# yl602019618/Reconstruction-of-PDE-without-Time-Label

Hardware: AMD Instinct MI355X
Metric: snapshot-bags/sec (train step) + rel-L2 drift error, 2D FPE 128² @1/2/4/8 GPU (higher is better)
Workload: dtype f32; 1 GPU; 2d_FPE train_fno.py NIOFP2D_FNO(2,3,100,25,3,12,32,2) (C), grid 128x128; per_gpu_batch=4, global_batch=4, T=100, bag_size=L=randint(50,T) with replacement, dataset_bags=4096, parallelism=dp1, optimizer=Adam lr 0.0005 (fused flat), launch=hip-graph per bag size L (all kernels replayed each step)

## Files before the change

include/blindno.h:

```cpp
#ifndef BLINDNO_H
#define BLINDNO_H

#include <stdint.h>

#ifdef __cplusplus
extern "C" {
#endif

typedef void* blindno_stream_t;

int blindno_abi_version(void);
const char* blindno_error_string(int code);


int blindno_lift_fwd(const float* in, const float* w0, const float* b0, float* x0,
                     int Bn, int N1, int N2, int Cin, int C, int P1, int P2,
                     blindno_stream_t stream);

int blindno_lift_bwd(const float* dx0, const float* in, const float* w0, float* d_in,
                     float* partial, int nchunk,
                     int Bn, int N1, int N2, int Cin, int C, int P1, int P2,
                     blindno_stream_t stream);
int blindno_lift_bwd_nchunk(int Bn, int N1, int N2);

int blindno_project_fwd(const float* z, const float* w1, const float* b1, const float* w2,
                        const float* b2, float* out, int Bn, int C, int P1, int P2, int Ho,
                        int Wo, int Hd, int Cout, int ostride, int ooff,
                        blindno_stream_t stream);

int blindno_project_bwd(const float* z, const float* w1, const float* b1, const float* w2,
                        const float* dout, float* dz, float* partial, int nchunk,
                        int Bn, int C, int P1, int P2, int Ho, int Wo, int Hd, int Cout,
                        int ostride, int ooff, int dout_div, blindno_stream_t stream);
int blindno_project_bwd_nchunk(int Bn, int Ho, int Wo);
int blindno_project_bwd_nchunk_heads(int Bg, int Ho, int Wo);
int blindno_project_bwd_w(const float* z, const float* w1, const float* b1, const float* w2,
                          const float* dout, const float* lscale, float* dz, float* partial,
                          int nchunk, int Bn, int C, int P1, int P2, int Ho, int Wo, int Hd,
                          int Cout, int ostride, int ooff, int dout_div, blindno_stream_t stream);

int64_t blindno_project_bag_stats_floats(int B, int Ho, int Wo);
int blindno_project_bag_bwd_nchunk(int B, int Ho, int Wo);
int blindno_project_bag_fwd(const float* z, const float* w1, const float* b1, const float* w2,
                            const float* b2, const float* lw, float* ubar, float* stats,
                            float* v, int B, int U, int C, int P1, int P2, int Ho, int Wo, int Hd,
                            blindno_stream_t stream);
int blindno_project_bag_bwd(const float* stats, const float* gs, const float* w2, const float* lw,
                            const float* v, float* dz, float* partial, int nchunk, int B, int U,
                            int C, int P1, int P2, int Ho, int Wo, int Hd,
                            blindno_stream_t stream);


int blindno_rowdft(const float* x, float* At, const float* Tp, int Bn, int C, int P1,
                   int P2, int m2, int act, blindno_stream_t stream);
int blindno_rowdft_crop(const float* x, float* At, const float* Tp, int Bn, int C, int P1,
                        int P2, int m2, int act, int N1v, int N2v, blindno_stream_t stream);

int blindno_colpass(const float* At, const float* Wt, float* Xs, float* Y, float* Z,
                    const float* FB, const float* GB, int Bn, int Ci, int Co, int P1, int m1,
                    int m2, int P2, int dir, blindno_stream_t stream);

int blindno_mix_wgrad_nsplit(int Bn, int Ci, int Co, int K1, int m2);
int blindno_mix_wgrad(const float* X, const float* G, float* dWt, float* partial, int nsplit,
                      int Bn, int Ci, int Co, int K1, int m2, blindno_stream_t stream);
int blindno_mix_wgrad_part(const float* X, const float* G, float* partial, int nsplit, int Gw,
                           int Bn, int Ci, int Co, int K1, int m2, blindno_stream_t stream);
int blindno_mix_wgrad_multi(const void* const* X, const void* const* G, void* const* out,
                            const int* shp, int njobs, blindno_stream_t stream);
int blindno_mix_wgrad_multi_u(const void* const* X, const void* const* G, void* const* out,
                              const int* shp, void* const* ud, const int* um1, int njobs,
                              blindno_stream_t stream);

int blindno_mix1d(const float* At, const float* Wt, float* Xs, float* Z, int Bn, int Ci,
                  int Co, int m, int P2, int dir, blindno_stream_t stream);

int blindno_rowidft_epi(const float* Z, const float* x, const float* wc, const float* bc,
                        float* z, const float* tb, int Bn, int C, int P1, int P2, int m2,
                        int act, blindno_stream_t stream);
int blindno_rowidft_epi_crop(const float* Z, const float* x, const float* wc, const float* bc,
                             float* z, const float* tb, int Bn, int C, int P1, int P2, int m2,
                             int act, int oN1, int oN2, blindno_stream_t stream);

int blindno_rowidft_bwd(const float* G, const float* dz, const float* wc, const float* xsrc,
                        float* dx, const float* tb, float* partial, int Bn, int C, int P1,
                        int P2, int m2, int act, blindno_stream_t stream);
int blindno_rowidft_bwd_crop(const float* G, const float* dz, const float* wc, const float* xsrc,
                             float* dx, const float* tb, float* partial, int Bn, int C, int P1,
                             int P2, int m2, int act, int dN1, int dN2, blindno_stream_t stream);
int blindno_rowidft_bwd_nchunk(int Bn, int C, int P1, int P2, int m2);
int blindno_set_rowfuse(int on);
int blindno_set_colfuse(int on);
int blindno_rowidft_bwd_rd(const float* G, const float* dz, const float* wc, const float* xsrc,
                           float* dx, const float* tb, float* partial, int Bn, int C, int P1,
                           int P2, int m2, int act, int dN1, int dN2, float* At, const float* Tp,
                           blindno_stream_t stream);
int blindno_rowidft_epi_rd(const float* Z, const float* x, const float* wc, const float* bc,
                           float* z, const float* tb, int Bn, int C, int P1, int P2, int m2,
                           int act, float* At, const float* Tp, int act_next,
                           blindno_stream_t stream);

int blindno_spectrum_tile_layout(int Bn, int C, int P1, int P2, int m2);


int blindno_rowdft_bag_lift(const float* X, const int* idx, const float* w0, const float* Gt,
                            float* At, const float* Tp, int B, int T, int L, int N1, int N2,
                            int C, int P1, int P2, int m2, blindno_stream_t stream);
int blindno_rowdft_bag_lift_dg(const float* X, const int* idx, const float* w0, const float* b0,
                               const float* Dg, float* At, const float* Tp, int B, int T, int L,
                               int N1, int N2, int C, int P1, int P2, int m2,
                               blindno_stream_t stream);

int blindno_rowidft_epi_lift(const float* Z, const float* X, const int* idx, const float* grid,
                             const float* w0, const float* b0, const float* wc, const float* bc,
                             float* z, const float* tb, int B, int T, int L, int N1, int N2,
                             int C, int P1, int P2, int m2, blindno_stream_t stream);
int blindno_rowidft_epi_lift_rd(const float* Z, const float* X, const int* idx, const float* grid,
                                const float* w0, const float* b0, const float* wc,
                                const float* bc, float* z, const float* tb, int B, int T, int L,
                                int N1, int N2, int C, int P1, int P2, int m2, float* At,
                                const float* Tp, int act_next, blindno_stream_t stream);

int blindno_rowidft_bwd_lift(const float* G, const float* dz, const float* X, const int* idx,
                             const float* grid, const float* w0, const float* b0, const float* wc,
                             const float* tb, float* partial, int B, int T, int L, int N1, int N2,
                             int C, int P1, int P2, int m2, blindno_stream_t stream);

int blindno_colspec_ok(int Bn, int C, int P1, int P2, int m1, int m2);
int blindno_colspec_nchunk(int C, int m2);
int blindno_colspec_bwd_nchunk(int Bn, int P1);
int blindno_rowdft_cd(const float* x, float* part, const float* Tp, const float* tab, int Bn, int C,
                      int P1, int P2, int m2, int act, int N1v, int N2v, blindno_stream_t stream);
int blindno_rowdft_bag_lift_cd(const float* X, const int* idx, float* part, const float* Tp,
                               const float* tab, int B, int T, int L, int N1, int N2, int P1,
                               int P2, int m2, blindno_stream_t stream);
int blindno_rowdft_bag_lift_cd_pack(const float* X, const int* idx, float* part, const float* Tp,
                                    const float* tab, int B, int T, int L, int N1, int N2, int P1,
                                    int P2, int m2, const void* const* w1s, const void* const* w2s,
                                    void* const* Wts, const int* shapes, int npk,
                                    blindno_stream_t stream);
int blindno_colmix(const float* part, int nbv, const float* Wt, float* Xsave, float* Y, int Bn, int C,
                   int Cp, int P1, int P2, int m1, int m2, int dir, const float* w0, const float* b0,
                   const float* Dg2, blindno_stream_t stream);
int blindno_rowidft_epi_zc(const float* Y, const float* x, const float* wc, const float* bc, float* z,
                           const float* tb, const float* tab, float* part, const float* Tp, int Bn,
                           int C, int P1, int P2, int m1, int m2, int act, int act_next, int oN1,
                           int oN2, blindno_stream_t stream);
int blindno_rowidft_epi_lift_zc(const float* Y, const float* X, const int* idx, const float* grid,
                                const float* w0, const float* b0, const float* wc, const float* bc,
                                float* z, const float* tb, const float* tab, float* part,
                                const float* Tp, int B, int T, int L, int N1, int N2, int C, int P1,
                                int P2, int m1, int m2, int act_next, blindno_stream_t stream);
int blindno_rowidft_bwd_zc(const float* Y, const float* dz, const float* wc, const float* xsrc,
                           float* dx, const float* tb, const float* tab, float* part,
                           const float* Tp, float* partial, int Bn, int C, int P1, int P2, int m1,
                           int m2, int act, int dN1, int dN2, blindno_stream_t stream);
int blindno_rowdft_cd_bag(const float* v, const float* ghat, const float* lw, int U, float* part,
                          const float* Tp, const float* tab, int Bn, int C, int P1, int P2, int m2,
                          int Ho, int Wo, blindno_stream_t stream);
int blindno_rowidft_bwd_zc_bag(const float* Y, const float* v, const float* ghat, const float* lw,
                               int U, const float* wc, const float* xsrc, float* dx, const float* tb,
                               const float* tab, float* part, const float* Tp, float* partial,
                               int Bn, int C, int P1, int P2, int m1, int m2, int act, int Ho, int Wo,
                               blindno_stream_t stream);
int blindno_rowidft_bwd_lift_zc_mix(const float* Y, const float* dz, const float* X, const int* idx,
                                    const float* grid, const float* w0, const float* b0,
                                    const float* wc, const float* tb, const float* tab,
                                    float* partial, int B, int T, int L, int N1, int N2, int C,
                                    int P1, int P2, int m1, int m2, const void* const* mX,
                                    const void* const* mG, void* const* mOut, const int* mshp,
                                    int nmj, blindno_stream_t stream);
int blindno_rowidft_bwd_lift_zc(const float* Y, const float* dz, const float* X, const int* idx,
                                const float* grid, const float* w0, const float* b0,
                                const float* wc, const float* tb, const float* tab, float* partial,
                                int B, int T, int L, int N1, int N2, int C, int P1, int P2, int m1,
                                int m2, blindno_stream_t stream);

int blindno_conv_wgrad(const float* dz, const float* x, float* partial, int nchunk, int Bn,
                       int C, int P1, int P2, int act, blindno_stream_t stream);
int blindno_conv_wgrad_nchunk(int Bn, int P1, int P2);

int blindno_reduce_partials(const float* partial, float* out, int nchunk, int np,
                            blindno_stream_t stream);

int blindno_reduce_partials_multi(const void* const* partials, void* const* outs,
                                  const int* nchunks, const int* nps, int nseg,
                                  blindno_stream_t stream);
int blindno_reduce_partials_pieces(const void* const* partials, void* const* outs,
                                   const int* nchunks, const int* nps, const int* e0s,
                                   const int* e1s, int nseg, blindno_stream_t stream);
int blindno_reduce_segs_limit(int what);
int blindno_reduce_partials_pieces_u(const void* const* partials, void* const* outs,
                                     const int* nchunks, const int* nps, const int* e0s,
                                     const int* e1s, const int* upks, void* const* ud,
                                     const int* ushp, int nseg, blindno_stream_t stream);
int blindno_finish_multi(const void* const* partials, void* const* outs, const int* nchunks,
                         const int* nps, const int* e0s, const int* e1s, const int* upks,
                         void* const* ud, const int* ushp, int nseg, const void* const* dWts,
                         void* const* dw1s, void* const* dw2s, const int* shapes, int nunp,
                         blindno_stream_t stream);
// ... 261 lines not shown
```

reconstruction-of-pde-without-time-label_amd/blindno/_lib.py:

```python
from __future__ import annotations

import ctypes
import os
import threading

import torch

_HERE = os.path.dirname(os.path.abspath(__file__))
LIB_PATH = os.environ.get("BLINDNO_LIB", os.path.join(_HERE, "libblindno.so"))

SIGNATURES = {
    "blindno_abi_version": "",
    "blindno_lift_fwd": "ppppiiiiiiis",
    "blindno_lift_bwd": "pppppiiiiiiiis",
    "blindno_project_fwd": "ppppppiiiiiiiiiis",
    "blindno_project_bwd": "pppppppiiiiiiiiiiiis",
    "blindno_rowdft": "pppiiiiiis",
    "blindno_rowdft_crop": "pppiiiiiiiis",
    "blindno_rowdft_bag_lift": "ppppppiiiiiiiiis",
    "blindno_rowdft_bag_lift_dg": "pppppppiiiiiiiiis",
    "blindno_rowidft_epi_lift": "ppppppppppiiiiiiiiis",
    "blindno_rowidft_bwd_lift": "ppppppppppiiiiiiiiis",
    "blindno_colpass": "pppppppiiiiiiiis",
    "blindno_colspec_ok": "iiiiii",
    "blindno_colspec_nchunk": "ii",
    "blindno_colspec_bwd_nchunk": "ii",
    "blindno_rowdft_cd": "ppppiiiiiiiis",
    "blindno_rowdft_bag_lift_cd": "pppppiiiiiiiis",
    "blindno_rowdft_bag_lift_cd_pack": "pppppiiiiiiiippppis",
    "blindno_colmix": "pipppiiiiiiiippps",
    "blindno_rowidft_epi_zc": "ppppppppp" + "iiiiiiiiii" + "s",
    "blindno_rowidft_epi_lift_zc": "ppppppppppppp" + "iiiiiiiiiii" + "s",
    "blindno_rowidft_bwd_zc": "pppppppppp" + "iiiiiiiii" + "s",
    "blindno_rowidft_bwd_lift_zc": "ppppppppppp" + "iiiiiiiiii" + "s",
    "blindno_rowidft_bwd_lift_zc_mix": "ppppppppppp" + "iiiiiiiiii" + "ppppi" + "s",
    "blindno_rowdft_cd_bag": "pppi" + "ppp" + "iiiiiii" + "s",
    "blindno_rowidft_bwd_zc_bag": "pppp" + "i" + "pppppppp" + "iiiiiiiii" + "s",
    "blindno_mix_wgrad": "ppppiiiiiis",
    "blindno_mix_wgrad_part": "pppiiiiiiis",
    "blindno_mix_wgrad_multi": "ppppis",
    "blindno_mix_wgrad_multi_u": "ppppppis",
    "blindno_mix1d": "ppppiiiiiis",
    "blindno_rowidft_epi": "ppppppiiiiiis",
    "blindno_rowidft_epi_crop": "pppppp" + "iiiiiiii" + "s",
    "blindno_rowidft_bwd": "pppppppiiiiiis",
    "blindno_rowidft_bwd_crop": "pppppppiiiiiiiis",
    "blindno_rowidft_bwd_rd": "pppppppiiiiiiiipps",
    "blindno_rowidft_epi_rd": "ppppppiiiiiippis",
    "blindno_rowidft_epi_lift_rd": "ppppppppppiiiiiiiiippis",
    "blindno_conv_wgrad": "pppiiiiiis",
    "blindno_reduce_partials": "ppiis",
    "blindno_spectrum_tile_layout": "iiiii",
    "blindno_pack_w2d": "pppiiiiis",
    "blindno_unpack_w2d": "pppiiiiis",
    "blindno_pack_w1d": "ppiiiis",
    "blindno_bagmean_fwd": "pppppiiiiis",
    "blindno_bagmean_bwd": "pppiiiiis",
    "blindno_mse": "pppplips",
    "blindno_mse_finish": "pilps",
    "blindno_mse_finish_acc": "pilpps",
    "blindno_mse_fwd": "ppplipppps",
    "blindno_rowsq": "pppiiiiiis",
    "blindno_adam": "pppplddffffs",
    "blindno_gpe_solve": "ppppddiiipppiiis",
    "blindno_trapz_rows": "ppppiis",
    "blindno_lift_bwd_nchunk": "iii",
    "blindno_conv_wgrad_nchunk": "iii",
    "blindno_rowidft_bwd_nchunk": "iiiii",
    "blindno_set_rowfuse": "i",
    "blindno_set_colfuse": "i",
    "blindno_project_bwd_nchunk": "iii",
    "blindno_project_bwd_nchunk_heads": "iii",
    "blindno_mix_wgrad_nsplit": "iiiii",
    "blindno_lift_fwd_g": "ppppiliiiiiiis",
    "blindno_lift_fwd_bag_g": "ppppiliiiiiiippppfs",
    "blindno_lift_bag_ok": "iiiiiiii",
    "blindno_lift_bwd_g": "pppppiiliiiiiiis",
    "blindno_lift_bwd_mix_g": "pppppiiliiiiiiippppiiis",
    "blindno_lift_bwd_bag_mix_g": "pppppiiliiiiiiippppiiippppffs",
    "blindno_project_fwd_g": "ppppppiliiiiiiiiiis",
    "blindno_project_bwd_g": "pppppppiiliiiiiiiiiis",
    "blindno_colpass_g": "pppppppiliiiiiiiis",
    "blindno_mix_wgrad_g": "ppppiiiiiiis",
    "blindno_rowidft_epi_g": "ppppppiliiiiiis",
    "blindno_rowidft_bwd_g": "ppppppiliiiiiis",
    "blindno_conv_wgrad_g": "pppiiiiiiis",
    "blindno_rowdft_wgrad_ok": "iiiii",
    "blindno_rowdft_wgrad_g": "pppppiippppiiiiiiiis",
    "blindno_bagmean_fwd_w": "pppppp" + "iiiii" + "s",
    "blindno_project_bwd_w": "pppppppp" + "i" + "iiiiiiiiiii" + "s",
    "blindno_project_bag_stats_floats": "iii",
    "blindno_project_bag_bwd_nchunk": "iii",
    "blindno_project_bag_fwd": "ppppppppp" + "iiiiiiii" + "s",
    "blindno_project_bag_bwd": "ppppppp" + "i" + "iiiiiiii" + "s",
    "blindno_pack_w2d_2": "ppppp" + "iiiii" + "s",
    "blindno_unpack_w2d_2": "ppppp" + "iiiii" + "s",
    "blindno_bn_act_nslices": "iii",
    "blindno_bn_act_fwd": "ppppppppiiiifffis",
    "blindno_bn_act_bwd": "pppppppppiiiifis",
    "blindno_gather_flat": "pppips",
    "blindno_gather_batch": "ppppipis",
    "blindno_reduce_partials_multi": "ppppis",
    "blindno_reduce_partials_pieces": "ppppppis",
    "blindno_reduce_partials_pieces_u": "pppppppppis",
    "blindno_reduce_segs_limit": "i",
    "blindno_finish_multi": "pppppppppippppis",
    "blindno_unpack_w2d_multi": "ppppis",
    "blindno_pack_w2d_multi": "ppppis",
    "blindno_fp_propagate": "pppiiiiiids",
    "blindno_bagattn_nchunk": "i",
    "blindno_bagattn_fwd": "pppppppp" + "iiii" + "s",
    "blindno_bagattn_bwd": "ppppppppppp" + "iiii" + "s",
    "blindno_conv2d_fwd": "pppp" + "iiiiiiiiiii" + "s",
    "blindno_conv2d_bwd_data": "ppp" + "iiiiiiiiiii" + "s",
    "blindno_conv2d_wgrad_nsplit": "iiiiiiiiiii",
    "blindno_conv2d_bwd_weight": "pppp" + "i" + "iiiiiiiiiii" + "s",
    "blindno_conv2d_fwd_nsplit": "iiiiiiiiiii",
    "blindno_conv2d_fwd_split": "ppppp" + "i" + "p" + "iiiiiiiiiii" + "s",
    "blindno_conv2d_bwd_data_nsplit": "iiiiiiiiiii",
    "blindno_conv2d_bwd_data_split": "pppp" + "i" + "p" + "iiiiiiiiiii" + "s",
    "blindno_conv2d_wscratch_floats": "i" + "iiiiiiiiiii",
    "blindno_spectral2d_tables_bytes": "iiii",
    "blindno_spectral2d_tables_init": "piiii",
    "blindno_spectral_conv2d_workspace_bytes": "iiiiiiii",
    "blindno_spectral_conv2d_saved_bytes": "iiiii",
    "blindno_spectral_conv2d_fwd": "ppppppp" + "iiiiiii" + "s",
    "blindno_spectral_conv2d_bwd": "ppppppppp" + "iiiiiii" + "s",
    "blindno_spectral1d_tables_bytes": "ii",
    "blindno_spectral1d_tables_init": "pii",
    "blindno_spectral_conv1d_workspace_bytes": "iiiiii",
    "blindno_spectral_conv1d_saved_bytes": "iii",
    "blindno_spectral_conv1d_fwd": "pppppp" + "iiiii" + "s",
    "blindno_spectral_conv1d_bwd": "ppppppp" + "iiiii" + "s",
    "blindno_dwconv_fwd": "pppp" + "iiiiii" + "s",
    "blindno_dwconv_bwd_data": "ppp" + "iiiiii" + "s",
    "blindno_dwconv_wgrad_nsplit": "iiii",
    "blindno_dwconv_bwd_weight": "pppp" + "i" + "iiiiii" + "s",
    "blindno_cnx_pw_fwd": "ppppppppp" + "iii" + "s",
    "blindno_cnx_pw_bwd_nblk": "iii",
    "blindno_cnx_pw_bwd": "pppppppppp" + "iiii" + "s",
    "blindno_maxpool_fwd": "ppp" + "iiiii" + "s",
    "blindno_maxpool_bwd": "ppp" + "iiiii" + "s",
    "blindno_convt_fwd": "pppp" + "iiiiiiiii" + "s",
    "blindno_convt_bwd_data": "ppp" + "iiiiiiiii" + "s",
    "blindno_convt_wgrad_nparts": "iii",
    "blindno_convt_bwd_weight": "pppp" + "iiiiiiiii" + "s",
    "blindno_tok_gram_nchunk": "l",
    "blindno_tok_attn_save_floats": "iil",
    "blindno_tok_attn_fwd": "ppppppp" + "iil" + "f" + "s",
    "blindno_tok_attn_bwd_scratch_floats": "ii",
    "blindno_tok_attn_bwd": "pppppppp" + "iil" + "s",
    "blindno_deeponet_bag_nblk": "i",
    "blindno_deeponet_bag_fwd": "pppppp" + "iiii" + "f" + "s",
    "blindno_deeponet_bag_bwd": "pppppppp" + "iiiii" + "f" + "s",
    "blindno_spectral3d_ok": "iiiiiiiii",
    "blindno_colpass3d": "ppppppp" + "iiiiiiiiii" + "s",
    "blindno_pack_w3d": "ppppp" + "iiiiiiii" + "s",
    "blindno_unpack_w3d": "ppppp" + "iiiiiiii" + "s",
    "blindno_lift3d_fwd": "pppp" + "iiiiiiiii" + "s",
    "blindno_lift3d_bwd_nchunk": "iiii",
    "blindno_lift3d_bwd": "ppppp" + "i" + "iiiiiiiii" + "s",
    "blindno_project3d_fwd": "pppppp" + "iiiiiiiiii" + "s",
    "blindno_project3d_bwd_nchunk": "iiii",
    "blindno_project3d_bwd": "ppppppp" + "i" + "iiiiiiiiii" + "s",
}

RET64 = {n for n in SIGNATURES if n.endswith(("_bytes", "_floats"))}

_CT = {"p": ctypes.c_void_p, "i": ctypes.c_int, "l": ctypes.c_int64, "f": ctypes.c_float,
       "d": ctypes.c_double, "s": ctypes.c_void_p}

_lock = threading.Lock()
_lib = None


class BlindnoError(RuntimeError):
    pass


def load():
    global _lib
    with _lock:
        if _lib is not None:
            return _lib
        if not os.path.exists(LIB_PATH):
            raise BlindnoError(
                f"libblindno.so not found at {LIB_PATH}; build it with "
                "`python reconstruction-of-pde-without-time-label_amd/build.py` "
                "(there is no CPU fallback)")
        lib = ctypes.CDLL(LIB_PATH)
        for name, sig in SIGNATURES.items():
            fn = getattr(lib, name)
            fn.argtypes = [_CT[c] for c in sig]
            fn.restype = ctypes.c_int64 if name in RET64 else ctypes.c_int
        lib.blindno_error_string.argtypes = [ctypes.c_int]
        lib.blindno_error_string.restype = ctypes.c_char_p
        _lib = lib
        return lib


def exported_symbols():
    return list(SIGNATURES) + ["blindno_error_string"]


def stream_ptr(device=None):
    return ctypes.c_void_p(torch.cuda.current_stream(device).cuda_stream)


class _TensorPtr(ctypes.c_void_p):
    __slots__ = ("tensor",)


def ptr(t):
    if t is None:
        return None
    p = _TensorPtr(t.data_ptr())
    p.tensor = t
    return p


_HOOKS = {}


def query(name, *args) -> int:
    return int(getattr(load(), name)(*args))


def call(name, *args):
    lib = load()
    hook = _HOOKS.get(name)
    if hook is not None:
        hook.before(args)
    rc = getattr(lib, name)(*args)
    if hook is not None:
        hook.after(args)
    if rc != 0:
        msg = lib.blindno_error_string(rc).decode(errors="replace")
        raise BlindnoError(f"{name} failed: hip error {rc} ({msg})")
    return rc
```

reconstruction-of-pde-without-time-label_amd/csrc/bagproj.hip:

```cpp
#include "common.h"
#include "blindno.h"
#include "gelu_pk.h"

using namespace blindno;
using namespace blindno::gelu_pk;

namespace {

typedef float f32x4 __attribute__((ext_vector_type(4)));

constexpr int kHd = 128;
constexpr int kNStat = 6;
constexpr int kTileF4 = (kHd / 16) * kNStat * 64;
constexpr int kMaxU = 1024;
#ifndef BAGPROJ_QUAD
#define BAGPROJ_QUAD 1
#endif
#ifndef BAGPROJ_FWD_WAVES
#define BAGPROJ_FWD_WAVES 3
#endif
#ifndef BAGPROJ_SETUP2
#define BAGPROJ_SETUP2 1
#endif

struct BagGeom {
  unsigned npts, S, Wo, P2, HW, C, U;
  FastDiv dS, dWo;
  __device__ __forceinline__ unsigned base(unsigned f) const {
    const unsigned b = dS.div(f), s = f - b * S;
    const unsigned h = dWo.div(s), w = s - h * Wo;
    return b * U * C * HW + h * P2 + w;
  }
};

#ifndef BAGPROJ_BWD_UNROLL
#define BAGPROJ_BWD_UNROLL 1
#endif
#ifndef BAGPROJ_SC
#define BAGPROJ_SC 8
#endif
constexpr int kSC2 = BAGPROJ_SC;

__device__ __forceinline__ float swap_sum32(float a, float b) {
  const auto r = __builtin_amdgcn_permlane32_swap(__float_as_uint(a), __float_as_uint(b), false, false);
  return __uint_as_float(r[0]) + __uint_as_float(r[1]);
}

__device__ __forceinline__ float swap_sum16(float a, float b) {
  const auto r = __builtin_amdgcn_permlane16_swap(__float_as_uint(a), __float_as_uint(b), false, false);
  return __uint_as_float(r[0]) + __uint_as_float(r[1]);
}

#ifndef BAGPROJ_PROBE
#define BAGPROJ_PROBE 0
#endif
#if BAGPROJ_PROBE
__device__ unsigned long long g_bagproj_probe[32768 * 8];
#define BP_MARK(i)                                                                          \
  do {                                                                                      \
    __builtin_amdgcn_sched_barrier(0);                                                      \
    const unsigned long long t_ = __builtin_amdgcn_s_memrealtime();                         \
    const int slot_ = blockIdx.x * 4 + (threadIdx.x >> 6);                                  \
    if ((threadIdx.x & 63) == 0 && slot_ < 32768) g_bagproj_probe[slot_ * 8 + (i)] = t_;    \
    __builtin_amdgcn_sched_barrier(0);                                                      \
  } while (0)
#else
#define BP_MARK(i) do {} while (0)
#endif
__global__ __launch_bounds__(256, BAGPROJ_FWD_WAVES) void bagproj_fwd_kernel(
    const float* __restrict__ z, const float* __restrict__ w1, const float* __restrict__ b1,
    const float* __restrict__ w2, const float* __restrict__ b2, const float* __restrict__ lw,
    float* __restrict__ ubar, float* __restrict__ stats, float* __restrict__ v, BagGeom g) {
  __shared__ float slw[kMaxU];
  __shared__ float zs[2][kSC2][16][4];
  __shared__ float zw[2][kSC2][16][4];
  __shared__ float vred[2][4][kSC2][64];
  __shared__ float zbr[4][64];
  __shared__ float vpart[16][4];
  __shared__ float vhalf[4];
  __shared__ float ured[4][16];
  __shared__ float2 swr[4][4][2][2][4];
  const int tid = threadIdx.x, lane = tid & 63;
  const int wave = uniform_int(tid >> 6);
  const int c16 = lane & 15, g4 = lane >> 4;
  const int C = (int)g.C, U = (int)g.U;
  BP_MARK(0);
  const int cs = (tid >> 4) & 3, ls = tid >> 6;
  const unsigned ntiles = (g.npts + 15) / 16;
  auto zload = [&](unsigned bo, bool ok, int ch, float (&zr)[kSC2 / 4]) {
#pragma unroll
    for (int i = 0; i < kSC2 / 4; ++i) {
      const int lg = ch * kSC2 + ls + 4 * i;
#if BAGPROJ_SETUP2
      const int lc = lg < U ? lg : U - 1, cc = cs < C ? cs : C - 1;
      const float zv = z[bo + (unsigned)(lc * C + cc) * g.HW];
      zr[i] = (ok && lg < U && cs < C) ? zv : 0.f;
#else
      zr[i] = (ok && lg < U && cs < C) ? z[bo + (unsigned)(lg * C + cs) * g.HW] : 0.f;
#endif
    }
  };
  float wa[2], bb[2][4], vloc[4] = {0.f, 0.f, 0.f, 0.f};
#if BAGPROJ_SETUP2
  __shared__ float sw1[kHd * 4], sb1[kHd], sw2[kHd];
  constexpr int kLwIt = kMaxU / 256;
  float lwv[kLwIt], w1v[2], b1v = 0.f, w2v = 0.f;
#pragma unroll
  for (int i = 0; i < kLwIt; ++i) {
    const int l = tid + 256 * i;
    lwv[i] = l < U ? (lw ? lw[l] : 1.0f / (float)U) : 0.f;
  }
#pragma unroll
  for (int i = 0; i < 2; ++i) w1v[i] = tid + 256 * i < kHd * C ? w1[tid + 256 * i] : 0.f;
  if (tid < kHd) {
    b1v = b1[tid];
    w2v = w2[tid];
  }
  float zfirst[kSC2 / 4];
  {
    const unsigned f = blockIdx.x * 16 + (unsigned)c16;
    const bool ok = f < g.npts;
    zload(g.base(ok ? f : 0u), ok, 0, zfirst);
  }
#pragma unroll
  for (int i = 0; i < kLwIt; ++i)
    if (tid + 256 * i < U) slw[tid + 256 * i] = lwv[i];
#pragma unroll
  for (int i = 0; i < 2; ++i)
    if (tid + 256 * i < kHd * C) sw1[tid + 256 * i] = w1v[i];
  if (tid < kHd) {
    sb1[tid] = b1v;
    sw2[tid] = w2v;
  }
  __syncthreads();
#pragma unroll
  for (int tt = 0; tt < 2; ++tt) {
    const int k0 = 16 * (2 * wave + tt);
    wa[tt] = g4 < C ? kK * sw1[(k0 + c16) * C + g4] : 0.f;
#pragma unroll
    for (int r = 0; r < 4; ++r) {
      const int k = k0 + 4 * g4 + r;
      bb[tt][r] = kK * sb1[k];
      if (c16 == 0) {
#pragma unroll
        for (int c = 0; c < 4; ++c) {
          const float wrv = c < C ? sw2[k] * sw1[k * C + c] : 0.f;
          vloc[c] += wrv;
          float2& e = swr[wave][g4][tt][r >> 1][c];
          if (r & 1) e.y = wrv; else e.x = wrv;
        }
      }
    }
  }
#else
  float zfirst[kSC2 / 4];
  for (int l = tid; l < U; l += 256) slw[l] = lw ? lw[l] : 1.0f / (float)U;
#pragma unroll
  for (int tt = 0; tt < 2; ++tt) {
    const int k0 = 16 * (2 * wave + tt);
    wa[tt] = g4 < C ? kK * w1[(k0 + c16) * C + g4] : 0.f;
#pragma unroll
    for (int r = 0; r < 4; ++r) {
      const int k = k0 + 4 * g4 + r;
      bb[tt][r] = kK * b1[k];
      if (c16 == 0) {
#pragma unroll
        for (int c = 0; c < 4; ++c) {
          const float wrv = c < C ? w2[k] * w1[k * C + c] : 0.f;
          vloc[c] += wrv;
          float2& e = swr[wave][g4][tt][r >> 1][c];
          if (r & 1) e.y = wrv; else e.x = wrv;
        }
      }
    }
  }
#endif
  if (c16 == 0) {
#pragma unroll
    for (int c = 0; c < 4; ++c) vpart[4 * wave + g4][c] = 0.5f * vloc[c];
  }
  __syncthreads();
  if (tid < 4) {
    float acc = 0.f;
    for (int j = 0; j < 16; ++j) acc += vpart[j][tid];
    vhalf[tid] = acc;
  }
#if !BAGPROJ_SETUP2
  float lsum = 0.f;
  for (int l = 0; l < U; ++l) lsum += slw[l];
  const float b2l = b2[0] * lsum;
#endif
  BP_MARK(1);

  const int nch = (U + kSC2 - 1) / kSC2;
  for (unsigned tile = blockIdx.x; tile < ntiles; tile += gridDim.x) {
    const unsigned f = tile * 16 + (unsigned)c16;
    const bool ok = f < g.npts;
    const unsigned bo = g.base(ok ? f : 0u);
    float zbp = 0.f;
    float zn[kSC2 / 4];
    auto load = [&](int ch) { zload(bo, ok, ch, zn); };
    auto store = [&](int ch, int buf) {
#pragma unroll
      for (int i = 0; i < kSC2 / 4; ++i) {
        const int l = ls + 4 * i, lg = ch * kSC2 + l;
        const float wv = zn[i] * slw[lg < U ? lg : 0];
        zs[buf][l][c16][cs] = zn[i];
        zw[buf][l][c16][cs] = wv;
        zbp += wv;
      }
    };
    auto vwrite = [&](int ch, int buf) {
#pragma unroll
      for (int i = 0; i < kSC2 / 4; ++i) {
        const int l = ls + 4 * i, lg = ch * kSC2 + l;
        if (ok && lg < U && cs < C)
          v[bo + (unsigned)(lg * C + cs) * g.HW] =
              (((vred[buf][0][l][lane] + vred[buf][1][l][lane]) + vred[buf][2][l][lane]) +
               vred[buf][3][l][lane]) + vhalf[cs];
      }
    };
    f32x2 A[2][2], S[2][2], Q[2][4][2];
#pragma unroll
    for (int tt = 0; tt < 2; ++tt)
#pragma unroll
      for (int i = 0; i < 2; ++i) {
        A[tt][i] = S[tt][i] = (f32x2){0.f, 0.f};
#pragma unroll
        for (int c = 0; c < 4; ++c) Q[tt][c][i] = (f32x2){0.f, 0.f};
      }
    if (BAGPROJ_SETUP2 && tile == blockIdx.x) {
#pragma unroll
      for (int i = 0; i < kSC2 / 4; ++i) zn[i] = zfirst[i];
    } else {
      load(0);
    }
    store(0, 0);
    if (nch > 1) load(1);
#if BAGPROJ_SETUP2
    float lsum = 0.f;
#endif
    __syncthreads();
    BP_MARK(2);
    for (int ch = 0; ch < nch; ++ch) {
      const int buf = ch & 1, l0 = ch * kSC2;
      const int nl = U - l0 < kSC2 ? U - l0 : kSC2;
      for (int l = 0; l < nl; ++l) {
        int zo;
        asm volatile("v_mov_b32 %0, 0" : "=v"(zo));
        const float4 zc = *reinterpret_cast<const float4*>(&zw[buf][l][c16][0]);
        const float az = zs[buf][l][c16][g4];
        const float lwl = slw[l0 + l];
        const f32x2 wl = splat2(lwl);
#if BAGPROJ_SETUP2
        lsum += lwl;
#endif
        f32x2 vp[4];
#if BAGPROJ_QUAD
        f32x2 hq[4], sq[4], eq[4];
#pragma unroll
        for (int tt = 0; tt < 2; ++tt) {
          f32x4 d = {bb[tt][0], bb[tt][1], bb[tt][2], bb[tt][3]};
          d = __builtin_amdgcn_mfma_f32_16x16x4f32(wa[tt], az, d, 0, 0, 0);
          hq[2 * tt] = (f32x2){d[0], d[1]};
          hq[2 * tt + 1] = (f32x2){d[2], d[3]};
        }
        norm_cdf_quad_pdf_centered(hq, sq, eq);
#endif
#pragma unroll
        for (int tt = 0; tt < 2; ++tt) {
#if !BAGPROJ_QUAD
          f32x4 d = {bb[tt][0], bb[tt][1], bb[tt][2], bb[tt][3]};
          d = __builtin_amdgcn_mfma_f32_16x16x4f32(wa[tt], az, d, 0, 0, 0);
          const f32x2 h[2] = {{d[0], d[1]}, {d[2], d[3]}};
#else
          const f32x2 h[2] = {hq[2 * tt], hq[2 * tt + 1]};
#endif
#pragma unroll
          for (int i = 0; i < 2; ++i) {
#if BAGPROJ_QUAD
            const f32x2 ep = eq[2 * tt + i], sg = sq[2 * tt + i];
#else
            f32x2 ep;
            const f32x2 sg = norm_cdf_pair_pdf_centered(h[i], ep);
#endif
            const f32x2 gd = pk_fma(h[i], ep, sg);
            A[tt][i] = pk_fma(wl, h[i] * sg, A[tt][i]);
            S[tt][i] = pk_fma(wl, gd, S[tt][i]);
            Q[tt][0][i] = pk_fma(gd, splat2(zc.x), Q[tt][0][i]);
            Q[tt][1][i] = pk_fma(gd, splat2(zc.y), Q[tt][1][i]);
            Q[tt][2][i] = pk_fma(gd, splat2(zc.z), Q[tt][2][i]);
            Q[tt][3][i] = pk_fma(gd, splat2(zc.w), Q[tt][3][i]);
            const float4* wq = reinterpret_cast<const float4*>(&swr[wave][g4][tt][i][0]) + zo;
            const float4 wq0 = wq[0], wq1 = wq[1];
            const f32x2 q0 = {wq0.x, wq0.y}, q1 = {wq0.z, wq0.w}, q2 = {wq1.x, wq1.y}, q3 = {wq1.z, wq1.w};
            if (tt == 0 && i == 0) {
              vp[0] = gd * q0; vp[1] = gd * q1; vp[2] = gd * q2; vp[3] = gd * q3;
            } else {
              vp[0] = pk_fma(gd, q0, vp[0]);
              vp[1] = pk_fma(gd, q1, vp[1]);
              vp[2] = pk_fma(gd, q2, vp[2]);
              vp[3] = pk_fma(gd, q3, vp[3]);
            }
          }
        }
        const float a = swap_sum32(vp[0].x + vp[0].y, vp[2].x + vp[2].y);
        const float b = swap_sum32(vp[1].x + vp[1].y, vp[3].x + vp[3].y);
        vred[buf][wave][l][lane] = swap_sum16(a, b);
      }
      if (ch + 1 < nch) {
        store(ch + 1, buf ^ 1);
        if (ch + 2 < nch) load(ch + 2);
      }
      if (ch >= 1) vwrite(ch - 1, buf ^ 1);
      __syncthreads();
    }
    vwrite(nch - 1, (nch - 1) & 1);
#if BAGPROJ_SETUP2
    const float b2l = b2[0] * lsum;
#endif
    zbr[ls][lane] = zbp;
    BP_MARK(3);
    __syncthreads();
    float4* st = reinterpret_cast<float4*>(stats) + (size_t)tile * kTileF4 + lane;
    float zb[4];
#pragma unroll
    for (int c = 0; c < 4; ++c)
      zb[c] = ((zbr[0][16 * c + c16] + zbr[1][16 * c + c16]) + zbr[2][16 * c + c16]) + zbr[3][16 * c + c16];
    float up = 0.f;
#pragma unroll
    for (int tt = 0; tt < 2; ++tt) {
      const int t = 2 * wave + tt;
      float av[4];
#pragma unroll
      for (int r = 0; r < 4; ++r) {
        const int k = 16 * t + 4 * g4 + r;
#if BAGPROJ_SETUP2
        float hb = sb1[k] * lsum;
#pragma unroll
        for (int c = 0; c < 4; ++c) hb = c < C ? fmaf(sw1[k * C + c], zb[c], hb) : hb;
#else
        float hb = b1[k] * lsum;
#pragma unroll
        for (int c = 0; c < 4; ++c) hb = c < C ? fmaf(w1[k * C + c], zb[c], hb) : hb;
#endif
        const float acc = r == 0 ? A[tt][0].x : (r == 1 ? A[tt][0].y : (r == 2 ? A[tt][1].x : A[tt][1].y));
        av[r] = fmaf(kInvK, acc, 0.5f * hb);
      }
      const float4 a4 = {av[0], av[1], av[2], av[3]};
      const int kb = 16 * t + 4 * g4;
#if BAGPROJ_SETUP2
      up += (sw2[kb] * a4.x + sw2[kb + 1] * a4.y) + (sw2[kb + 2] * a4.z + sw2[kb + 3] * a4.w);
#else
      up += (w2[kb] * a4.x + w2[kb + 1] * a4.y) + (w2[kb + 2] * a4.z + w2[kb + 3] * a4.w);
#endif
      st[(t * kNStat + 0) * 64] = a4;
      const float hs = 0.5f * lsum;
      st[(t * kNStat + 1) * 64] = (float4){S[tt][0].x + hs, S[tt][0].y + hs, S[tt][1].x + hs, S[tt][1].y + hs};
#pragma unroll
      for (int c = 0; c < 4; ++c) {
        const float hz = 0.5f * zb[c];
        st[(t * kNStat + 2 + c) * 64] =
            (float4){Q[tt][c][0].x + hz, Q[tt][c][0].y + hz, Q[tt][c][1].x + hz, Q[tt][c][1].y + hz};
      }
    }
    up += __shfl_xor(up, 16, 64);
    up += __shfl_xor(up, 32, 64);
    if (g4 == 0) ured[wave][c16] = up;
    __syncthreads();
    if (tid < 16 && ok) ubar[f] = (((ured[0][tid] + ured[1][tid]) + ured[2][tid]) + ured[3][tid]) + b2l;
  }
  BP_MARK(4);
#if BAGPROJ_PROBE
  if ((threadIdx.x & 63) == 0) {
    const int slot_ = blockIdx.x * 4 + (threadIdx.x >> 6);
    if (slot_ < 32768) {
      g_bagproj_probe[slot_ * 8 + 5] = __builtin_amdgcn_s_getreg((31 << 11) | 4);
      g_bagproj_probe[slot_ * 8 + 6] = __builtin_amdgcn_s_getreg((31 << 11) | 20);
    }
  }
#endif
}
#if BAGPROJ_PROBE
BLINDNO_API int blindno_bagproj_probe_read(unsigned long long* dst, int n) {
  return (int)hipMemcpyFromSymbol(dst, HIP_SYMBOL(g_bagproj_probe),
                                  sizeof(unsigned long long) * (size_t)n, 0, hipMemcpyDeviceToHost);
}
#endif

__global__ __launch_bounds__(256) void bagproj_bwd_kernel(
    const float* __restrict__ stats, const float* __restrict__ gs, const float* __restrict__ w2,
    const float* __restrict__ lw, const float* __restrict__ v, float* __restrict__ dz,
    float* __restrict__ partial, BagGeom g) {
  constexpr int kJ = kTileF4 / 256;
  __shared__ float slw[kMaxU];
  __shared__ float4 red[kJ * 4][4];
  __shared__ float sgs;
  const int tid = threadIdx.x, lane = tid & 63, c16 = lane & 15;
  const int C = (int)g.C, U = (int)g.U;
  for (int l = tid; l < U; l += 256) slw[l] = lw ? lw[l] : 1.0f / (float)U;
  __syncthreads();
  float4 acc[kJ];
#pragma unroll
  for (int j = 0; j < kJ; ++j) acc[j] = (float4){0.f, 0.f, 0.f, 0.f};
  float gsum = 0.f;
  const int cw = tid >> 6, p64 = tid & 63;
  const unsigned ntiles = (g.npts + 15) / 16;
  const unsigned ntg = (ntiles + 3) / 4;
  for (unsigned tg = blockIdx.x; tg < ntg; tg += gridDim.x) {
    if (dz) {
      const unsigned f = tg * 64 + (unsigned)p64;
      if (f < g.npts && cw < C) {
        const float gh = gs[f];
        const unsigned bo = g.base(f) + (unsigned)cw * g.HW;
        const unsigned ls = (unsigned)C * g.HW;
        int l = 0;
        for (; l + 3 < U; l += 4) {
          float vv[4];
#pragma unroll
          for (int i = 0; i < 4; ++i) vv[i] = v[bo + (unsigned)(l + i) * ls];
#pragma unroll
          for (int i = 0; i < 4; ++i) dz[bo + (unsigned)(l + i) * ls] = slw[l + i] * gh * vv[i];
        }
        for (; l < U; ++l) dz[bo + (unsigned)l * ls] = slw[l] * gh * v[bo + (unsigned)l * ls];
      }
    }
#pragma unroll BAGPROJ_BWD_UNROLL
    for (int t4 = 0; t4 < 4; ++t4) {
      const unsigned tile = tg * 4 + (unsigned)t4;
      if (tile >= ntiles) break;
      const unsigned f = tile * 16 + (unsigned)c16;
      const float gh = f < g.npts ? gs[f] : 0.f;
      const float4* st = reinterpret_cast<const float4*>(stats) + (size_t)tile * kTileF4 + tid;
      float4 sv[kJ];
#pragma unroll
      for (int j = 0; j < kJ; ++j) sv[j] = st[256 * j];
      if (tid < 16) gsum += gh;
#pragma unroll
      for (int j = 0; j < kJ; ++j) {
        acc[j].x = fmaf(gh, sv[j].x, acc[j].x);
        acc[j].y = fmaf(gh, sv[j].y, acc[j].y);
        acc[j].z = fmaf(gh, sv[j].z, acc[j].z);
        acc[j].w = fmaf(gh, sv[j].w, acc[j].w);
      }
    }
  }
#pragma unroll
  for (int j = 0; j < kJ; ++j) {
#pragma unroll
    for (int m = 1; m <= 8; m <<= 1) {
      acc[j].x += __shfl_xor(acc[j].x, m, 64);
      acc[j].y += __shfl_xor(acc[j].y, m, 64);
      acc[j].z += __shfl_xor(acc[j].z, m, 64);
      acc[j].w += __shfl_xor(acc[j].w, m, 64);
    }
    if (c16 == 0) red[(tid >> 6) + 4 * j][(tid >> 4) & 3] = acc[j];
  }
  if (tid < 64) {
    float s = gsum;
#pragma unroll
    for (int m = 1; m <= 8; m <<= 1) s += __shfl_xor(s, m, 64);
    if (tid == 0) sgs = s;
  }
  __syncthreads();
  float lsum = 0.f;
#pragma unroll 8
  for (int l = 0; l < U; ++l) lsum += slw[l];
  const int np_ = kHd * C + 2 * kHd + 1;
  float* pp = partial + (size_t)blockIdx.x * np_;
  for (int e = tid; e < np_; e += 256) {
    float val;
    int k, comp;
    if (e < kHd * C) {
      k = e / C;
      comp = 2 + e % C;
    } else if (e < kHd * C + kHd) {
      k = e - kHd * C;
      comp = 1;
    } else if (e < kHd * C + 2 * kHd) {
      k = e - kHd * C - kHd;
      comp = 0;
    } else {
      pp[e] = sgs * lsum;
      continue;
    }
    const float4 q = red[(k >> 4) * kNStat + comp][(k >> 2) & 3];
    const int r = k & 3;
    val = r == 0 ? q.x : (r == 1 ? q.y : (r == 2 ? q.z : q.w));
    pp[e] = comp == 0 ? val : w2[k] * val;
  }
}

bool bag_geom(int B, int U, int C, int P1, int P2, int Ho, int Wo, int Hd, BagGeom& g) {
  if (B < 1 || U < 1 || U > kMaxU || C < 1 || C > 4 || Hd != kHd || Ho < 1 || Wo < 1 || Ho > P1 ||
      Wo > P2)
    return false;
  if ((int64_t)B * U * C * P1 * P2 >= INT32_MAX || (int64_t)B * Ho * Wo >= INT32_MAX) return false;
  g.npts = (unsigned)(B * Ho * Wo);
  g.S = (unsigned)(Ho * Wo);
  g.Wo = (unsigned)Wo;
  g.P2 = (unsigned)P2;
  g.HW = (unsigned)(P1 * P2);
  g.C = (unsigned)C;
  g.U = (unsigned)U;
  g.dS = FastDiv::make(g.S);
  g.dWo = FastDiv::make(g.Wo);
  return true;
}

}

BLINDNO_API int64_t blindno_project_bag_stats_floats(int B, int Ho, int Wo) {
  return ((int64_t)B * Ho * Wo + 15) / 16 * (int64_t)kTileF4 * 4;
}

#ifndef BAGPROJ_BWD_BLOCKS
#define BAGPROJ_BWD_BLOCKS 1024
#endif
BLINDNO_API int blindno_project_bag_bwd_nchunk(int B, int Ho, int Wo) {
  const int64_t tiles = ((int64_t)B * Ho * Wo + 15) / 16;
  return (int)(tiles < 1 ? 1 : (tiles > BAGPROJ_BWD_BLOCKS ? BAGPROJ_BWD_BLOCKS : tiles));
}

BLINDNO_API int blindno_project_bag_fwd(const float* z, const float* w1, const float* b1,
                                        const float* w2, const float* b2, const float* lw,
                                        float* ubar, float* stats, float* v, int B, int U, int C,
                                        int P1, int P2, int Ho, int Wo, int Hd, void* stream) {
  BagGeom g;
  if (!bag_geom(B, U, C, P1, P2, Ho, Wo, Hd, g) || !z || !ubar || !stats || !v)
    return (int)hipErrorInvalidValue;
  const unsigned ntiles = (g.npts + 15) / 16;
  bagproj_fwd_kernel<<<ntiles, 256, 0, (hipStream_t)stream>>>(z, w1, b1, w2, b2, lw, ubar, stats,
                                                               v, g);
  return (int)hipGetLastError();
}

BLINDNO_API int blindno_project_bag_bwd(const float* stats, const float* gs, const float* w2,
                                        const float* lw, const float* v, float* dz,
                                        float* partial, int nchunk, int B, int U, int C, int P1,
                                        int P2, int Ho, int Wo, int Hd, void* stream) {
  BagGeom g;
  if (!bag_geom(B, U, C, P1, P2, Ho, Wo, Hd, g) || !stats || !gs || (dz && !v) || !partial ||
      nchunk < 1)
    return (int)hipErrorInvalidValue;
  bagproj_bwd_kernel<<<nchunk, 256, 0, (hipStream_t)stream>>>(stats, gs, w2, lw, v, dz, partial, g);
  return (int)hipGetLastError();
}
```

Baseline: 3667 snapshot-bags/s.

## Pipeline bag projection forward across tiles and chunks with optional persistent grid

Restructures the bag projection forward kernel into a single flattened loop over (tile, chunk) pairs. The next chunk's loads and the previous tile's stats/ubar epilogue overlap with current compute, using double-buffered shared reductions. Adds a grid-size entry point that can launch an occupancy-sized persistent grid. The default launch still uses one block per tile, so the cross-tile overlap only matters when a smaller grid is requested. Extra state and registers may reduce occupancy.

```diff
diff --git a/include/blindno.h b/include/blindno.h
--- a/include/blindno.h
+++ b/include/blindno.h
@@ -45,6 +45,12 @@
                             const float* b2, const float* lw, float* ubar, float* stats,
                             float* v, int B, int U, int C, int P1, int P2, int Ho, int Wo, int Hd,
                             blindno_stream_t stream);
+int64_t blindno_project_bag_fwd_workspace_bytes(void);
+int blindno_project_bag_fwd_grid(const float* z, const float* w1, const float* b1,
+                                 const float* w2, const float* b2, const float* lw, float* ubar,
+                                 float* stats, float* v, int B, int U, int C, int P1, int P2,
+                                 int Ho, int Wo, int Hd, float* workspace, int nwg,
+                                 blindno_stream_t stream);
 int blindno_project_bag_bwd(const float* stats, const float* gs, const float* w2, const float* lw,
                             const float* v, float* dz, float* partial, int nchunk, int B, int U,
                             int C, int P1, int P2, int Ho, int Wo, int Hd,
diff --git a/reconstruction-of-pde-without-time-label_amd/blindno/_lib.py b/reconstruction-of-pde-without-time-label_amd/blindno/_lib.py
--- a/reconstruction-of-pde-without-time-label_amd/blindno/_lib.py
+++ b/reconstruction-of-pde-without-time-label_amd/blindno/_lib.py
@@ -92,6 +92,8 @@
     "blindno_project_bag_stats_floats": "iii",
     "blindno_project_bag_bwd_nchunk": "iii",
     "blindno_project_bag_fwd": "ppppppppp" + "iiiiiiii" + "s",
+    "blindno_project_bag_fwd_workspace_bytes": "",
+    "blindno_project_bag_fwd_grid": "ppppppppp" + "iiiiiiii" + "pi" + "s",
     "blindno_project_bag_bwd": "ppppppp" + "i" + "iiiiiiii" + "s",
     "blindno_pack_w2d_2": "ppppp" + "iiiii" + "s",
     "blindno_unpack_w2d_2": "ppppp" + "iiiii" + "s",
diff --git a/reconstruction-of-pde-without-time-label_amd/csrc/bagproj.hip b/reconstruction-of-pde-without-time-label_amd/csrc/bagproj.hip
--- a/reconstruction-of-pde-without-time-label_amd/csrc/bagproj.hip
+++ b/reconstruction-of-pde-without-time-label_amd/csrc/bagproj.hip
@@ -1,3 +1,6 @@
+#include <atomic>
+#include <climits>
+
 #include "common.h"
 #include "blindno.h"
 #include "gelu_pk.h"
@@ -19,8 +22,8 @@
 #ifndef BAGPROJ_FWD_WAVES
 #define BAGPROJ_FWD_WAVES 3
 #endif
-#ifndef BAGPROJ_SETUP2
-#define BAGPROJ_SETUP2 1
+#ifndef BAGPROJ_FWD_GRID
+#define BAGPROJ_FWD_GRID INT_MAX
 #endif
 
 struct BagGeom {
@@ -75,10 +78,10 @@
   __shared__ float zs[2][kSC2][16][4];
   __shared__ float zw[2][kSC2][16][4];
   __shared__ float vred[2][4][kSC2][64];
-  __shared__ float zbr[4][64];
+  __shared__ float zbr[2][4][64];
   __shared__ float vpart[16][4];
   __shared__ float vhalf[4];
-  __shared__ float ured[4][16];
+  __shared__ float ured[2][4][16];
   __shared__ float2 swr[4][4][2][2][4];
   const int tid = threadIdx.x, lane = tid & 63;
   const int wave = uniform_int(tid >> 6);
@@ -91,17 +94,12 @@
 #pragma unroll
     for (int i = 0; i < kSC2 / 4; ++i) {
       const int lg = ch * kSC2 + ls + 4 * i;
-#if BAGPROJ_SETUP2
       const int lc = lg < U ? lg : U - 1, cc = cs < C ? cs : C - 1;
       const float zv = z[bo + (unsigned)(lc * C + cc) * g.HW];
       zr[i] = (ok && lg < U && cs < C) ? zv : 0.f;
-#else
-      zr[i] = (ok && lg < U && cs < C) ? z[bo + (unsigned)(lg * C + cs) * g.HW] : 0.f;
-#endif
     }
   };
   float wa[2], bb[2][4], vloc[4] = {0.f, 0.f, 0.f, 0.f};
-#if BAGPROJ_SETUP2
   __shared__ float sw1[kHd * 4], sb1[kHd], sw2[kHd];
   constexpr int kLwIt = kMaxU / 256;
   float lwv[kLwIt], w1v[2], b1v = 0.f, w2v = 0.f;
@@ -116,12 +114,14 @@
     b1v = b1[tid];
     w2v = w2[tid];
   }
-  float zfirst[kSC2 / 4];
-  {
-    const unsigned f = blockIdx.x * 16 + (unsigned)c16;
-    const bool ok = f < g.npts;
-    zload(g.base(ok ? f : 0u), ok, 0, zfirst);
-  }
+  auto tile_ok = [&](unsigned tile) { return tile * 16 + (unsigned)c16 < g.npts; };
+  auto tile_bo = [&](unsigned tile) {
+    const unsigned f = tile * 16 + (unsigned)c16;
+    return g.base(f < g.npts ? f : 0u);
+  };
+  float zn[kSC2 / 4];
+  unsigned boC = tile_bo(blockIdx.x);
+  zload(boC, tile_ok(blockIdx.x), 0, zn);
 #pragma unroll
   for (int i = 0; i < kLwIt; ++i)
     if (tid + 256 * i < U) slw[tid + 256 * i] = lwv[i];
@@ -152,29 +152,6 @@
       }
     }
   }
-#else
-  float zfirst[kSC2 / 4];
-  for (int l = tid; l < U; l += 256) slw[l] = lw ? lw[l] : 1.0f / (float)U;
-#pragma unroll
-  for (int tt = 0; tt < 2; ++tt) {
-    const int k0 = 16 * (2 * wave + tt);
-    wa[tt] = g4 < C ? kK * w1[(k0 + c16) * C + g4] : 0.f;
-#pragma unroll
-    for (int r = 0; r < 4; ++r) {
-      const int k = k0 + 4 * g4 + r;
-      bb[tt][r] = kK * b1[k];
-      if (c16 == 0) {
-#pragma unroll
-        for (int c = 0; c < 4; ++c) {
-          const float wrv = c < C ? w2[k] * w1[k * C + c] : 0.f;
-          vloc[c] += wrv;
-          float2& e = swr[wave][g4][tt][r >> 1][c];
-          if (r & 1) e.y = wrv; else e.x = wrv;
-        }
-      }
-    }
-  }
-#endif
   if (c16 == 0) {
 #pragma unroll
     for (int c = 0; c < 4; ++c) vpart[4 * wave + g4][c] = 0.5f * vloc[c];
@@ -185,42 +162,45 @@
     for (int j = 0; j < 16; ++j) acc += vpart[j][tid];
     vhalf[tid] = acc;
   }
-#if !BAGPROJ_SETUP2
-  float lsum = 0.f;
-  for (int l = 0; l < U; ++l) lsum += slw[l];
-  const float b2l = b2[0] * lsum;
-#endif
   BP_MARK(1);
 
+  const float b2v = b2[0];
   const int nch = (U + kSC2 - 1) / kSC2;
-  for (unsigned tile = blockIdx.x; tile < ntiles; tile += gridDim.x) {
-    const unsigned f = tile * 16 + (unsigned)c16;
-    const bool ok = f < g.npts;
-    const unsigned bo = g.base(ok ? f : 0u);
-    float zbp = 0.f;
-    float zn[kSC2 / 4];
-    auto load = [&](int ch) { zload(bo, ok, ch, zn); };
-    auto store = [&](int ch, int buf) {
-#pragma unroll
-      for (int i = 0; i < kSC2 / 4; ++i) {
-        const int l = ls + 4 * i, lg = ch * kSC2 + l;
-        const float wv = zn[i] * slw[lg < U ? lg : 0];
-        zs[buf][l][c16][cs] = zn[i];
-        zw[buf][l][c16][cs] = wv;
-        zbp += wv;
-      }
-    };
-    auto vwrite = [&](int ch, int buf) {
-#pragma unroll
-      for (int i = 0; i < kSC2 / 4; ++i) {
-        const int l = ls + 4 * i, lg = ch * kSC2 + l;
-        if (ok && lg < U && cs < C)
-          v[bo + (unsigned)(lg * C + cs) * g.HW] =
-              (((vred[buf][0][l][lane] + vred[buf][1][l][lane]) + vred[buf][2][l][lane]) +
-               vred[buf][3][l][lane]) + vhalf[cs];
-      }
-    };
-    f32x2 A[2][2], S[2][2], Q[2][4][2];
+  const unsigned stride = gridDim.x;
+  auto advance = [&](unsigned& tile, int& ch, unsigned& bo) {
+    if (ch + 1 < nch) {
+      ++ch;
+      return;
+    }
+    ch = 0;
+    tile = tile + stride < ntiles ? tile + stride : ntiles;
+    bo = tile_bo(tile);
+  };
+  float zbp = 0.f;
+  auto store = [&](int ch, int buf) {
+#pragma clang fp contract(off)
+#pragma unroll
+    for (int i = 0; i < kSC2 / 4; ++i) {
+      const int l = ls + 4 * i, lg = ch * kSC2 + l;
+      const float lwv_ = slw[lg < U ? lg : 0];
+      const float wv = zn[i] * lwv_;
+      zs[buf][l][c16][cs] = zn[i];
+      zw[buf][l][c16][cs] = wv;
+      zbp = ch == 0 ? zbp + wv : fmaf(zn[i], lwv_, zbp);
+    }
+  };
+  auto vwrite = [&](unsigned bo, bool ok, int ch, int buf) {
+#pragma unroll
+    for (int i = 0; i < kSC2 / 4; ++i) {
+      const int l = ls + 4 * i, lg = ch * kSC2 + l;
+      if (ok && lg < U && cs < C)
+        v[bo + (unsigned)(lg * C + cs) * g.HW] =
+            (((vred[buf][0][l][lane] + vred[buf][1][l][lane]) + vred[buf][2][l][lane]) +
+             vred[buf][3][l][lane]) + vhalf[cs];
+    }
+  };
+  f32x2 A[2][2], S[2][2], Q[2][4][2];
+  auto zero_acc = [&]() {
 #pragma unroll
     for (int tt = 0; tt < 2; ++tt)
 #pragma unroll
@@ -229,21 +209,85 @@
 #pragma unroll
         for (int c = 0; c < 4; ++c) Q[tt][c][i] = (f32x2){0.f, 0.f};
       }
-    if (BAGPROJ_SETUP2 && tile == blockIdx.x) {
-#pragma unroll
-      for (int i = 0; i < kSC2 / 4; ++i) zn[i] = zfirst[i];
-    } else {
-      load(0);
-    }
-    store(0, 0);
-    if (nch > 1) load(1);
-#if BAGPROJ_SETUP2
-    float lsum = 0.f;
-#endif
-    __syncthreads();
-    BP_MARK(2);
-    for (int ch = 0; ch < nch; ++ch) {
-      const int buf = ch & 1, l0 = ch * kSC2;
+  };
+  zero_acc();
+  unsigned tP = ntiles, tC = blockIdx.x, boP = 0u;
+  int chP = 0, chC = 0;
+  store(0, 0);
+  unsigned t1 = tC, bo1 = boC;
+  int ch1 = chC;
+  advance(t1, ch1, bo1);
+  zload(bo1, tile_ok(t1), ch1, zn);
+  unsigned t2 = t1, bo2 = bo1;
+  int ch2 = ch1;
+  advance(t2, ch2, bo2);
+  float lsum = 0.f;
+  float lsumU = 0.f;
+  int buf = 0, par = 0;
+  bool upend = false;
+  unsigned tU = 0u;
+  int parU = 0;
+  auto ubar_store = [&]() {
+    const unsigned fu = tU * 16 + (unsigned)tid;
+    if (tid < 16 && fu < g.npts)
+      ubar[fu] = fmaf(b2v, lsumU,
+                      ((ured[parU][0][tid] + ured[parU][1][tid]) + ured[parU][2][tid]) + ured[parU][3][tid]);
+  };
+  __syncthreads();
+  BP_MARK(2);
+  for (;;) {
+    if (upend) {
+      ubar_store();
+      upend = false;
+    }
+    if (chC == 0 && tP < ntiles) {
+      lsumU = lsum;
+      float4* st = reinterpret_cast<float4*>(stats) + (size_t)tP * kTileF4 + lane;
+      float zb[4];
+#pragma unroll
+      for (int c = 0; c < 4; ++c)
+        zb[c] = ((zbr[par][0][16 * c + c16] + zbr[par][1][16 * c + c16]) + zbr[par][2][16 * c + c16]) +
+                zbr[par][3][16 * c + c16];
+      float up = 0.f;
+#pragma unroll
+      for (int tt = 0; tt < 2; ++tt) {
+        const int t = 2 * wave + tt;
+        float av[4];
+#pragma unroll
+        for (int r = 0; r < 4; ++r) {
+          const int k = 16 * t + 4 * g4 + r;
+          float hb = sb1[k] * lsum;
+#pragma unroll
+          for (int c = 0; c < 4; ++c) hb = c < C ? fmaf(sw1[k * C + c], zb[c], hb) : hb;
+          const float acc = r == 0 ? A[tt][0].x : (r == 1 ? A[tt][0].y : (r == 2 ? A[tt][1].x : A[tt][1].y));
+          av[r] = fmaf(kInvK, acc, 0.5f * hb);
+        }
+        const float4 a4 = {av[0], av[1], av[2], av[3]};
+        const int kb = 16 * t + 4 * g4;
+        up += (sw2[kb] * a4.x + sw2[kb + 1] * a4.y) + (sw2[kb + 2] * a4.z + sw2[kb + 3] * a4.w);
+        st[(t * kNStat + 0) * 64] = a4;
+        const float hs = 0.5f * lsum;
+        st[(t * kNStat + 1) * 64] = (float4){S[tt][0].x + hs, S[tt][0].y + hs, S[tt][1].x + hs, S[tt][1].y + hs};
+#pragma unroll
+        for (int c = 0; c < 4; ++c) {
+          const float hz = 0.5f * zb[c];
+          st[(t * kNStat + 2 + c) * 64] =
+              (float4){Q[tt][c][0].x + hz, Q[tt][c][0].y + hz, Q[tt][c][1].x + hz, Q[tt][c][1].y + hz};
+        }
+      }
+      up += __shfl_xor(up, 16, 64);
+      up += __shfl_xor(up, 32, 64);
+      if (g4 == 0) ured[par][wave][c16] = up;
+      upend = true;
+      tU = tP;
+      parU = par;
+      par ^= 1;
+      zero_acc();
+      lsum = 0.f;
+    }
+    if (tC >= ntiles) break;
+    {
+      const int l0 = chC * kSC2;
       const int nl = U - l0 < kSC2 ? U - l0 : kSC2;
       for (int l = 0; l < nl; ++l) {
         int zo;
@@ -252,9 +296,7 @@
         const float az = zs[buf][l][c16][g4];
         const float lwl = slw[l0 + l];
         const f32x2 wl = splat2(lwl);
-#if BAGPROJ_SETUP2
         lsum += lwl;
-#endif
         f32x2 vp[4];
 #if BAGPROJ_QUAD
         f32x2 hq[4], sq[4], eq[4];
@@ -308,67 +350,26 @@
         const float b = swap_sum32(vp[1].x + vp[1].y, vp[3].x + vp[3].y);
         vred[buf][wave][l][lane] = swap_sum16(a, b);
       }
-      if (ch + 1 < nch) {
-        store(ch + 1, buf ^ 1);
-        if (ch + 2 < nch) load(ch + 2);
-      }
-      if (ch >= 1) vwrite(ch - 1, buf ^ 1);
-      __syncthreads();
-    }
-    vwrite(nch - 1, (nch - 1) & 1);
-#if BAGPROJ_SETUP2
-    const float b2l = b2[0] * lsum;
-#endif
-    zbr[ls][lane] = zbp;
-    BP_MARK(3);
+    }
+    if (ch1 == 0) {
+      zbr[par][ls][lane] = zbp;
+      zbp = 0.f;
+    }
+    store(ch1, buf ^ 1);
+    zload(bo2, tile_ok(t2), ch2, zn);
+    vwrite(boP, tile_ok(tP), chP, buf ^ 1);
     __syncthreads();
-    float4* st = reinterpret_cast<float4*>(stats) + (size_t)tile * kTileF4 + lane;
-    float zb[4];
-#pragma unroll
-    for (int c = 0; c < 4; ++c)
-      zb[c] = ((zbr[0][16 * c + c16] + zbr[1][16 * c + c16]) + zbr[2][16 * c + c16]) + zbr[3][16 * c + c16];
-    float up = 0.f;
-#pragma unroll
-    for (int tt = 0; tt < 2; ++tt) {
-      const int t = 2 * wave + tt;
-      float av[4];
-#pragma unroll
-      for (int r = 0; r < 4; ++r) {
-        const int k = 16 * t + 4 * g4 + r;
-#if BAGPROJ_SETUP2
-        float hb = sb1[k] * lsum;
-#pragma unroll
-        for (int c = 0; c < 4; ++c) hb = c < C ? fmaf(sw1[k * C + c], zb[c], hb) : hb;
-#else
-        float hb = b1[k] * lsum;
-#pragma unroll
-        for (int c = 0; c < 4; ++c) hb = c < C ? fmaf(w1[k * C + c], zb[c], hb) : hb;
-#endif
-        const float acc = r == 0 ? A[tt][0].x : (r == 1 ? A[tt][0].y : (r == 2 ? A[tt][1].x : A[tt][1].y));
-        av[r] = fmaf(kInvK, acc, 0.5f * hb);
-      }
-      const float4 a4 = {av[0], av[1], av[2], av[3]};
-      const int kb = 16 * t + 4 * g4;
-#if BAGPROJ_SETUP2
-      up += (sw2[kb] * a4.x + sw2[kb + 1] * a4.y) + (sw2[kb + 2] * a4.z + sw2[kb + 3] * a4.w);
-#else
-      up += (w2[kb] * a4.x + w2[kb + 1] * a4.y) + (w2[kb + 2] * a4.z + w2[kb + 3] * a4.w);
-#endif
-      st[(t * kNStat + 0) * 64] = a4;
-      const float hs = 0.5f * lsum;
-      st[(t * kNStat + 1) * 64] = (float4){S[tt][0].x + hs, S[tt][0].y + hs, S[tt][1].x + hs, S[tt][1].y + hs};
-#pragma unroll
-      for (int c = 0; c < 4; ++c) {
-        const float hz = 0.5f * zb[c];
-        st[(t * kNStat + 2 + c) * 64] =
-            (float4){Q[tt][c][0].x + hz, Q[tt][c][0].y + hz, Q[tt][c][1].x + hz, Q[tt][c][1].y + hz};
-      }
-    }
-    up += __shfl_xor(up, 16, 64);
-    up += __shfl_xor(up, 32, 64);
-    if (g4 == 0) ured[wave][c16] = up;
+    tP = tC, chP = chC, boP = boC;
+    tC = t1, chC = ch1, boC = bo1;
+    t1 = t2, ch1 = ch2, bo1 = bo2;
+    advance(t2, ch2, bo2);
+    buf ^= 1;
+  }
+  BP_MARK(3);
+  vwrite(boP, tile_ok(tP), chP, buf ^ 1);
+  if (upend) {
     __syncthreads();
-    if (tid < 16 && ok) ubar[f] = (((ured[0][tid] + ured[1][tid]) + ured[2][tid]) + ured[3][tid]) + b2l;
+    ubar_store();
   }
   BP_MARK(4);
 #if BAGPROJ_PROBE
@@ -526,12 +527,49 @@
                                         const float* w2, const float* b2, const float* lw,
                                         float* ubar, float* stats, float* v, int B, int U, int C,
                                         int P1, int P2, int Ho, int Wo, int Hd, void* stream) {
+  return blindno_project_bag_fwd_grid(z, w1, b1, w2, b2, lw, ubar, stats, v, B, U, C, P1, P2, Ho,
+                                      Wo, Hd, nullptr, BAGPROJ_FWD_GRID, stream);
+}
+
+static int bagproj_fwd_slots() {
+  constexpr int kMaxDev = 64;
+  static std::atomic<int> cache[kMaxDev];
+  int dev = 0;
+  if (hipGetDevice(&dev) != hipSuccess) return 0;
+  if (dev >= 0 && dev < kMaxDev) {
+    const int c = cache[dev].load(std::memory_order_relaxed);
+    if (c > 0) return c;
+  }
+  int per_cu = 0, cus = 0;
+  if (hipOccupancyMaxActiveBlocksPerMultiprocessor(&per_cu, bagproj_fwd_kernel, 256, 0) != hipSuccess ||
+      hipDeviceGetAttribute(&cus, hipDeviceAttributeMultiprocessorCount, dev) != hipSuccess ||
+      per_cu < 1 || cus < 1)
+    return 0;
+  if (dev >= 0 && dev < kMaxDev) cache[dev].store(per_cu * cus, std::memory_order_relaxed);
+  return per_cu * cus;
+}
+
+BLINDNO_API int64_t blindno_project_bag_fwd_workspace_bytes(void) { return 0; }
+
+BLINDNO_API int blindno_project_bag_fwd_grid(const float* z, const float* w1, const float* b1,
+                                             const float* w2, const float* b2, const float* lw,
+                                             float* ubar, float* stats, float* v, int B, int U,
+                                             int C, int P1, int P2, int Ho, int Wo, int Hd,
+                                             float* workspace, int nwg, void* stream) {
   BagGeom g;
-  if (!bag_geom(B, U, C, P1, P2, Ho, Wo, Hd, g) || !z || !ubar || !stats || !v)
+  if (!bag_geom(B, U, C, P1, P2, Ho, Wo, Hd, g) || !z || !w1 || !b1 || !w2 || !b2 || !ubar || !stats || !v)
     return (int)hipErrorInvalidValue;
+  (void)workspace;
   const unsigned ntiles = (g.npts + 15) / 16;
-  bagproj_fwd_kernel<<<ntiles, 256, 0, (hipStream_t)stream>>>(z, w1, b1, w2, b2, lw, ubar, stats,
-                                                               v, g);
+  unsigned grid;
+  if (nwg > 0) {
+    grid = (unsigned)nwg < ntiles ? (unsigned)nwg : ntiles;
+  } else {
+    const int slots = bagproj_fwd_slots();
+    if (slots < 1) return (int)hipErrorInvalidValue;
+    grid = (unsigned)slots < ntiles ? (unsigned)slots : ntiles;
+  }
+  bagproj_fwd_kernel<<<grid, 256, 0, (hipStream_t)stream>>>(z, w1, b1, w2, b2, lw, ubar, stats, v, g);
   return (int)hipGetLastError();
 }
 
```

Measured after the change: 3674 snapshot-bags/s (median of 4 runs). Within noise of the previous version (+0.2%).
